# peterrum/deal-and-ceed-on-gpu

Measured on AMD Instinct MI355X. Metric: BP5 DoFs/sec per CG iter (p=4, ~1e8 DoFs) + % HBM roofline at 1/2/4/8 GPUs, higher is better.
Workload: dtype f64

## Files before the change

deal-and-ceed-on-gpu_amd/csrc/bp5_device.hpp:

```cpp
#pragma once
#include "bp5_internal.hpp"
#include "bp5_kernels.hpp"

#include <hip/hip_runtime.h>
#include <rccl/rccl.h>

#include <algorithm>
#include <cmath>
#include <cstdio>
#include <cstdlib>
#include <cstring>
#include <map>
#include <memory>
#include <tuple>
#include <vector>

using namespace bp5;

#define HIP_TRY(expr)                                                                                              \
  do {                                                                                                             \
    hipError_t e_ = (expr);                                                                                        \
    if (e_ != hipSuccess)                                                                                          \
      return fail(e_ == hipErrorNoDevice || e_ == hipErrorInvalidDevice ? BP5_ERR_NO_DEVICE : BP5_ERR_HIP,         \
                  std::string(#expr) + ": " + hipGetErrorString(e_));                                              \
// ... 776 lines not shown
      return fail(BP5_ERR_INVALID, "variant 59 needs the whole cell range"); }
    BP5_CASE(4, 57) { if (c0 == 0 && c1 == mf->n_cells) return LAUNCH_COLL(launch_block_t, 4, (32, BLK_SEQ), coef, src, dst, overwrite);
      return fail(BP5_ERR_INVALID, "variant 57 needs the whole cell range"); }
    BP5_CASE(4, 58) { if (c0 == 0 && c1 == mf->n_cells) return LAUNCH_COLL(launch_block_t, 4, (32, BLK_SINGLE | BLK_SEQ | BLK_NTM), coef, src, dst, overwrite);
      return fail(BP5_ERR_INVALID, "variant 58 needs the whole cell range"); }
#ifdef BP5_TIMING_BUILDS
    BP5_CASE(4, 99) return launch_block_t<4, false, 32, BLK_DEFAULT | BLK_STAMPS>(mf, call, coef, src, dst, true);
#endif
    BP5_CASE(4, 52) { if (c0 == 0 && c1 == mf->n_cells) return LAUNCH_COLL(launch_block_t, 4, (32, BLK_SINGLE), coef, src, dst, overwrite);
      return fail(BP5_ERR_INVALID, "variant 52 needs the whole cell range"); }
    BP5_CASE(4, 53) { if (c0 == 0 && c1 == mf->n_cells) return LAUNCH_COLL(launch_block_t, 4, (25, BLK_SINGLE), coef, src, dst, overwrite);
      return fail(BP5_ERR_INVALID, "variant 53 needs the whole cell range"); }
#ifdef BP5_TIMING_BUILDS
    BP5_CASE(4, 64) return launch_block_t<4, false, 32, BLK_DEFAULT | BLK_LATT>(mf, call, coef, src, dst, true);
    BP5_CASE(4, 65) return launch_block_t<4, false, 32, BLK_DEFAULT | BLK_LATT | 33554432>(mf, call, coef, src, dst, true);
    BP5_CASE(4, 66) return launch_block_t<4, false, 32, BLK_DEFAULT | BLK_LATT | 134217728>(mf, call, coef, src, dst, true);
    BP5_CASE(4, 87) return launch_block_t<4, false, 32, BLK_SINGLE | BLK_SEQ | BLK_RUNS | 65536>(mf, call, coef, src, dst, true);
    BP5_CASE(4, 91) return launch_block_t<4, false, 32, BLK_SINGLE | BLK_SEQ | BLK_RUNS | 1>(mf, call, coef, src, dst, true);
    BP5_CASE(4, 93) return launch_block_t<4, false, 32, BLK_SINGLE | BLK_SEQ | BLK_RUNS | 2>(mf, call, coef, src, dst, true);
    BP5_CASE(4, 95) return launch_block_t<4, false, 32, BLK_SINGLE | BLK_SEQ | BLK_RUNS | 4>(mf, call, coef, src, dst, true);
    BP5_CASE(4, 97) return launch_block_t<4, false, 32, BLK_STAMPS>(mf, call, coef, src, dst, true);
    BP5_CASE(4, 98) return launch_block_t<4, false, 32, BLK_STAMPS | BLK_SINGLE>(mf, call, coef, src, dst, true);
    BP5_CASE(4, 92) return launch_block_t<4, false, 32, BLK_SINGLE | 1>(mf, call, coef, src, dst, true);
    BP5_CASE(4, 96) return launch_block_t<4, false, 32, BLK_SINGLE | 5>(mf, call, coef, src, dst, true);
#endif
    BLOCK_CASE(5, 50, 36, 4, true);
    BLOCK_CASE(6, 50, 49, 4, false);
    BLOCK_CASE(7, 50, 64, 4, false);
    BLOCK_CASE(8, 50, 81, 4, false);
#ifdef BP5_TIMING_BUILDS
#define BABL_CASE(M) BP5_CASE(4, 60 + (M)) return launch_block_t<4, false, 25, M>(mf, call, coef, src, dst, true)
// ... 32 lines not shown
```

deal-and-ceed-on-gpu_amd/csrc/bp5_kernels.hpp:

```cpp
#pragma once
#include <hip/hip_runtime.h>
#include <stdint.h>
#include <type_traits>

namespace bp5 {

template <int n>
struct ShapeArg {
  double N[n * n];
  double D[n * n];
};

template <int n>
__host__ __device__ constexpr int coef_off(int qi, int ab)
{
  return (qi < 2 * (n / 2)) ? (qi / 2) * (2 * n * n) + 2 * ab + (qi & 1) : (n / 2) * (2 * n * n) + ab;
}
typedef double bp5_d2u __attribute__((ext_vector_type(2), aligned(8)));
template <int n, bool NT = false>
__device__ __forceinline__ void load_pencil(const double *base, int ab, double (&S)[n])
{
#pragma unroll
  for (int m = 0; m < n / 2; ++m) {
    const bp5_d2u *q = reinterpret_cast<const bp5_d2u *>(base + m * (2 * n * n) + 2 * ab);
    const bp5_d2u v = NT ? __builtin_nontemporal_load(q) : *q;
    S[2 * m] = v.x;
    S[2 * m + 1] = v.y;
  }
  if constexpr (n & 1) S[n - 1] = NT ? __builtin_nontemporal_load(base + (n / 2) * (2 * n * n) + ab) : base[(n / 2) * (2 * n * n) + ab];
}

typedef float bp5_f2u __attribute__((ext_vector_type(2), aligned(4)));
template <int n, bool NT = false>
__device__ __forceinline__ void load_pencil(const float *base, int ab, float (&S)[n])
{
#pragma unroll
  for (int m = 0; m < n / 2; ++m) {
    const bp5_f2u *q = reinterpret_cast<const bp5_f2u *>(base + m * (2 * n * n) + 2 * ab);
    const bp5_f2u v = NT ? __builtin_nontemporal_load(q) : *q;
    S[2 * m] = v.x;
    S[2 * m + 1] = v.y;
  }
  if constexpr (n & 1) S[n - 1] = NT ? __builtin_nontemporal_load(base + (n / 2) * (2 * n * n) + ab) : base[(n / 2) * (2 * n * n) + ab];
}
constexpr int BLK_F32M = 536870912;
template <int ABL> using metric_t = typename std::conditional<(ABL & BLK_F32M) != 0, float, double>::type;

template <int n, bool NT = false>
__device__ __forceinline__ void load_pencil_pair(const double *base, int ab, int m, double &s0, double &s1)
{
  const bp5_d2u *q = reinterpret_cast<const bp5_d2u *>(base + m * (2 * n * n) + 2 * ab);
  const bp5_d2u v = NT ? __builtin_nontemporal_load(q) : *q;
  s0 = v.x;
  s1 = v.y;
}
template <int n, bool NT = false>
__device__ __forceinline__ double load_pencil_tail(const double *base, int ab)
{
  return NT ? __builtin_nontemporal_load(base + (n / 2) * (2 * n * n) + ab) : base[(n / 2) * (2 * n * n) + ab];
}

struct ApplyArgs {
  const uint32_t *l2g;
  const double *coef;
  const double *src;
  double *dst;
  uint64_t plane_stride;
  uint64_t cell_stride;
  uint32_t cell_begin, cell_end;
  uint32_t n_teams;
  uint32_t teams_per_xcd;
  const double *gcell;
  uint32_t n_cells_total;
  const uint32_t *hang_mask;
// ... 203 lines not shown
#pragma unroll
  for (int k = 0; k < n; ++k) u[k] = (ABL & 4) ? 1e-9 * idx[k] : a.src[idx[k]];
  uint32_t hmask = 0;
  if constexpr ((ABL & 2097152) != 0) {
    hmask = a.hang_mask[cell];
    pencil_hang_resolve<n, TW, false, L>(hmask, a.hang_I, u, T, a_, b_, active);
  }

  if constexpr (ABL & 131072) {
    if (active) {
#pragma unroll
      for (int k = 0; k < n; ++k) a.dst[cell * n3 + k * n2 + abm] = u[k];
    }
  }
  using MT = metric_t<ABL>;
  const MT *cf = reinterpret_cast<const MT *>(a.coef) + cell * a.cell_stride;
  constexpr bool AFFINE = (ABL & 1024) != 0;
  constexpr bool HELM = (ABL & 8388608) != 0;
  static_assert(!HELM || (PF && !AFFINE), "Helmholtz build: prefetched planes, six-plane geometry");
  static_assert((ABL & BLK_F32M) == 0 || (!HELM && !AFFINE), "FP32 metric planes: Poisson operator, six-plane geometry");
  constexpr int NPL = HELM ? 7 : 6;
  MT S[(PF && !AFFINE) ? NPL : 1][n];
  double um[HELM ? n : 1];
  double Gc[6] = {0, 0, 0, 0, 0, 0};
  if constexpr (AFFINE) {
    load_pencil<n>(cf, abm, S[0]);
#pragma unroll
    for (int pl = 0; pl < 6; ++pl) Gc[pl] = a.gcell[(uint64_t)pl * a.n_cells_total + cell];
  } else if constexpr (PF) {
#pragma unroll
    for (int pl = 0; pl < NPL; ++pl) {
      if constexpr (ABL & 2) {
#pragma unroll
        for (int i = 0; i < n; ++i) S[pl][i] = 1.0 + pl + i + 1e-3 * abm;
      } else
        load_pencil<n, (ABL & 256) != 0>(cf + pl * a.plane_stride, abm, S[pl]);
    }
  }

  double g0[n], g1[n], g2[n];
  if constexpr (ABL & 8) {
#pragma unroll
    for (int i = 0; i < n; ++i) { g0[i] = u[i]; g1[i] = 2.0 * u[i]; g2[i] = 3.0 * u[i]; }
  } else if constexpr (!COLL) {
    double aN[n], aD[n];
    MV_N(sh.N, u, aN);
    MV_D(sh.D, u, aD);
    if (active) {
#pragma unroll
      for (int k = 0; k < n; ++k) { TL(0, k, b_, a_) = aN[k]; TL(1, k, b_, a_) = aD[k]; }
    }
    team_sync<TW>();
// ... 49 lines not shown
    if constexpr (HELM) {
#pragma unroll
      for (int i = 0; i < n; ++i) um[i] = r1[i];
    }
  }

#pragma unroll
  for (int i = 0; i < n; ++i) {
    double s00, s11, s22, s01, s02, s12;
    if constexpr (AFFINE) {
      const double sc = S[0][i];
      s00 = sc * Gc[0]; s11 = sc * Gc[1]; s22 = sc * Gc[2]; s01 = sc * Gc[3]; s02 = sc * Gc[4]; s12 = sc * Gc[5];
    } else if constexpr (PF) {
      s00 = S[0][i]; s11 = S[1][i]; s22 = S[2][i]; s01 = S[3][i]; s02 = S[4][i]; s12 = S[5][i];
    } else {
      s00 = cf[0 * a.plane_stride + coef_off<n>(i, abm)];
      s11 = cf[1 * a.plane_stride + coef_off<n>(i, abm)];
      s22 = cf[2 * a.plane_stride + coef_off<n>(i, abm)];
      s01 = cf[3 * a.plane_stride + coef_off<n>(i, abm)];
      s02 = cf[4 * a.plane_stride + coef_off<n>(i, abm)];
      s12 = cf[5 * a.plane_stride + coef_off<n>(i, abm)];
    }
    const double x0 = g0[i], x1 = g1[i], x2 = g2[i];
    g0[i] = s00 * x0 + s01 * x1 + s02 * x2;
    g1[i] = s01 * x0 + s11 * x1 + s12 * x2;
    g2[i] = s02 * x0 + s12 * x1 + s22 * x2;
    if constexpr (HELM) um[i] *= S[6][i];
  }

  double y[n];
  if constexpr (ABL & 8) {
#pragma unroll
    for (int i = 0; i < n; ++i) y[i] = g0[i] + g1[i] + g2[i];
  } else if constexpr (!COLL) {
    double e1[n], e2[n], e3[n];
    MV_DT(sh.D, g0, e1);
// ... 162 lines not shown

    uint32_t idx[n];
    double u[n];
    idx[0] = linked ? idx_carry : idxN[0];
    u[0] = linked ? u_carry : uN[0];
#pragma unroll
    for (int k = 1; k < n; ++k) { idx[k] = idxN[k]; u[k] = uN[k]; }
    u_carry = u[n - 1];
    idx_carry = idx[n - 1];
    {
      const uint32_t *l2g_n = a.l2g + (uint64_t)(e_next & 0x3fffffffu) * n3 + abm;
#pragma unroll
      for (int k = 0; k < n; ++k) idxN[k] = l2g_n[k * n2];
    }

    const double *cf = a.coef + cell * a.cell_stride;
    constexpr bool AFFINE = (ABL & 1024) != 0;
    double S[(PF && !AFFINE) ? 6 : 1][n];
    double Gc[6] = {0, 0, 0, 0, 0, 0};
    if constexpr (AFFINE) {
      load_pencil<n>(cf, abm, S[0]);
#pragma unroll
      for (int pl = 0; pl < 6; ++pl) Gc[pl] = a.gcell[(uint64_t)pl * a.n_cells_total + cell];
    } else if constexpr (PF) {
#pragma unroll
      for (int pl = 0; pl < 6; ++pl) {
        if constexpr (ABL & 2) {
#pragma unroll
          for (int i = 0; i < n; ++i) S[pl][i] = 1.0 + pl + i + 1e-3 * abm;
        } else
          load_pencil<n, (ABL & 256) != 0>(cf + pl * a.plane_stride, abm, S[pl]);
      }
    }

    double g0[n], g1[n], g2[n];
    if constexpr (ABL & 8) {
#pragma unroll
      for (int i = 0; i < n; ++i) { g0[i] = u[i]; g1[i] = 2.0 * u[i]; g2[i] = 3.0 * u[i]; }
    } else if constexpr (!COLL) {
      double aN[n], aD[n];
      MV_N(sh.N, u, aN);
      MV_D(sh.D, u, aD);
      if (active) {
#pragma unroll
        for (int k = 0; k < n; ++k) { TL(0, k, b_, a_) = aN[k]; TL(1, k, b_, a_) = aD[k]; }
      }
      team_sync<TW>();
// ... 47 lines not shown
      MV_D(sh.D, r1, g0);
    }

#pragma unroll
    for (int k = 0; k < n; ++k) uN[k] = a.src[idxN[k]];

#pragma unroll
    for (int i = 0; i < n; ++i) {
      double s00, s11, s22, s01, s02, s12;
      if constexpr (AFFINE) {
        const double sc = S[0][i];
        s00 = sc * Gc[0]; s11 = sc * Gc[1]; s22 = sc * Gc[2]; s01 = sc * Gc[3]; s02 = sc * Gc[4]; s12 = sc * Gc[5];
      } else if constexpr (PF) {
        s00 = S[0][i]; s11 = S[1][i]; s22 = S[2][i]; s01 = S[3][i]; s02 = S[4][i]; s12 = S[5][i];
      } else {
        s00 = cf[0 * a.plane_stride + coef_off<n>(i, abm)];
        s11 = cf[1 * a.plane_stride + coef_off<n>(i, abm)];
        s22 = cf[2 * a.plane_stride + coef_off<n>(i, abm)];
        s01 = cf[3 * a.plane_stride + coef_off<n>(i, abm)];
        s02 = cf[4 * a.plane_stride + coef_off<n>(i, abm)];
        s12 = cf[5 * a.plane_stride + coef_off<n>(i, abm)];
      }
      const double x0 = g0[i], x1 = g1[i], x2 = g2[i];
      g0[i] = s00 * x0 + s01 * x1 + s02 * x2;
      g1[i] = s01 * x0 + s11 * x1 + s12 * x2;
      g2[i] = s02 * x0 + s12 * x1 + s22 * x2;
    }

    double y[n];
    if constexpr (ABL & 8) {
#pragma unroll
      for (int i = 0; i < n; ++i) y[i] = g0[i] + g1[i] + g2[i];
    } else if constexpr (!COLL) {
      double e1[n], e2[n], e3[n];
      MV_DT(sh.D, g0, e1);
      MV_NT(sh.N, g1, e2);
// ... 106 lines not shown
  const int abm = ab < n2 ? ab : ab % n2;
  const int a_ = abm % n, b_ = abm / n;
  double *T = lds + (c < CPT ? c : 0) * L::CS;
#define TL(f, k, j, i) T[(f) * (n * L::PS) + (k) * L::PS + (j) * L::RS + (i)]

  const uint32_t o0 = tp.off[team];
  const int m = (int)(tp.off[team + 1] - o0);
  uint32_t gidx[MAXU];
#pragma unroll
  for (int r = 0; r < MAXU; ++r) {
    const int i = t + r * TEAM;
    gidx[r] = i < m ? tp.dofs[o0 + i] : 0u;
  }
  const int my_round = tp.cell_round[cell];
  const int n_rounds = tp.team_rounds[team];
  const double *cf = a.coef + cell * a.cell_stride;
  constexpr bool AFFINE = (ABL & 1024) != 0;
  double S[(PF && !AFFINE) ? 6 : 1][n];
  double Gc[6] = {0, 0, 0, 0, 0, 0};
  if constexpr (AFFINE) {
    load_pencil<n>(cf, abm, S[0]);
#pragma unroll
    for (int pl = 0; pl < 6; ++pl) Gc[pl] = a.gcell[(uint64_t)pl * a.n_cells_total + cell];
  } else if constexpr (PF) {
#pragma unroll
    for (int pl = 0; pl < 6; ++pl) load_pencil<n>(cf + pl * a.plane_stride, abm, S[pl]);
  }
  uint16_t ps[n];
  const uint16_t *pos_c = tp.pos + cell * n3 + abm;
#pragma unroll
  for (int k = 0; k < n; ++k) ps[k] = pos_c[k * n2];
  double u[n];
  if constexpr (ABL & 32) {
    const uint32_t *l2g_c = a.l2g + cell * n3 + abm;
    uint32_t idx[n];
#pragma unroll
    for (int k = 0; k < n; ++k) idx[k] = l2g_c[k * n2];
#pragma unroll
    for (int k = 0; k < n; ++k) u[k] = a.src[idx[k]];
  } else if constexpr (ABL & 4) {
#pragma unroll
// ... 59 lines not shown
    double r1[n];
#pragma unroll
    for (int i = 0; i < n; ++i) { r1[i] = TL(0, b_, a_, i); g1[i] = TL(1, b_, a_, i); g2[i] = TL(2, b_, a_, i); }
    MV_D(sh.D, r1, g0);
  }

#pragma unroll
  for (int i = 0; i < n; ++i) {
    double s00, s11, s22, s01, s02, s12;
    if constexpr (AFFINE) {
      const double sc = S[0][i];
      s00 = sc * Gc[0]; s11 = sc * Gc[1]; s22 = sc * Gc[2]; s01 = sc * Gc[3]; s02 = sc * Gc[4]; s12 = sc * Gc[5];
    } else if constexpr (PF) {
      s00 = S[0][i]; s11 = S[1][i]; s22 = S[2][i]; s01 = S[3][i]; s02 = S[4][i]; s12 = S[5][i];
    } else {
      s00 = cf[0 * a.plane_stride + coef_off<n>(i, abm)]; s11 = cf[1 * a.plane_stride + coef_off<n>(i, abm)]; s22 = cf[2 * a.plane_stride + coef_off<n>(i, abm)];
      s01 = cf[3 * a.plane_stride + coef_off<n>(i, abm)]; s02 = cf[4 * a.plane_stride + coef_off<n>(i, abm)]; s12 = cf[5 * a.plane_stride + coef_off<n>(i, abm)];
    }
    const double x0 = g0[i], x1 = g1[i], x2 = g2[i];
    g0[i] = s00 * x0 + s01 * x1 + s02 * x2;
    g1[i] = s01 * x0 + s11 * x1 + s12 * x2;
    g2[i] = s02 * x0 + s12 * x1 + s22 * x2;
  }

  double y[n];
  if constexpr (!COLL) {
    double e1[n], e2[n], e3[n];
    MV_DT(sh.D, g0, e1);
    MV_NT(sh.N, g1, e2);
    MV_NT(sh.N, g2, e3);
    __syncthreads();
    if (active) {
// ... 257 lines not shown
  {
    r.active = lane_ok && exists && !(r.ent >> 31);
    const uint64_t cell = r.ent & 0x7fffffffu;
    if constexpr (LATT) r.cpos = bp.cell_pos[cell];
    else if constexpr (PACK) load_pencil_idx<n, uint16_t>(bp.packed + cell * n3, abm, r.ps);
    else {
      load_pencil_idx<n, uint32_t>(bp.gidx + cell * n3, abm, r.idx);
      load_pencil_idx<n, uint16_t>(bp.pos + cell * n3, abm, r.ps);
    }
    r.round = bp.cell_round[cell];
    if constexpr (HANG) r.mask = a.hang_mask[cell];
    if constexpr (!SINGLE) issue_metric(a, r, abm);
  }
  static __device__ __forceinline__ void issue_metric_roll(const ApplyArgs &a, uint32_t ent, int abm, double (&S)[NPL][n])
  {
    const double *cf = a.coef + (uint64_t)(ent & 0x7fffffffu) * a.cell_stride;
#pragma unroll
    for (int pl = 0; pl < NPL; ++pl) {
      if constexpr (ABL & 2) {
#pragma unroll
        for (int i = 0; i < n; ++i) S[pl][i] = 1.0 + pl + i;
      } else
        load_pencil<n, (ABL & 32768) != 0>(cf + pl * a.plane_stride, abm, S[pl]);
    }
  }
  static __device__ __forceinline__ void issue_metric(const ApplyArgs &a, R &r, int abm)
  {
    if constexpr (ROLL) return;
    const uint64_t cell = r.ent & 0x7fffffffu;
    const MT *cf = reinterpret_cast<const MT *>(a.coef) + cell * a.cell_stride;
    if constexpr (AFFINE) {
      load_pencil<n>(cf, abm, r.S[0]);
#pragma unroll
      for (int pl = 0; pl < 6; ++pl) r.Gc[pl] = a.gcell[(uint64_t)pl * a.n_cells_total + cell];
    } else {
#ifdef BP5_TIMING_BUILDS
      if constexpr ((ABL & 33554432) != 0 && (n & 1)) {
        const uint64_t cell0 = (uint64_t)__builtin_amdgcn_readfirstlane((int)cell);
        const int lane = (int)(threadIdx.x & 63u);
#pragma unroll
        for (int pl = 0; pl < NPL; ++pl) {
          const double *base = a.coef + pl * a.plane_stride + ((cell0 * a.cell_stride) & ~(uint64_t)15);
#pragma unroll
          for (int m = 0; m < n / 2; ++m) {
            const bp5_d2u v = *reinterpret_cast<const bp5_d2u *>(base + (m * 64 + lane) * 2);
            r.S[pl][2 * m] = v.x;
            r.S[pl][2 * m + 1] = v.y;
          }
          r.S[pl][n - 1] = r.S[pl][0] + 1.0;
        }
        return;
      }
      if constexpr ((ABL & 134217728) != 0 && (n & 1) && NPL == 6) {
#pragma unroll
        for (int pl = 0; pl < NPL; ++pl) {
#pragma unroll
          for (int m = 0; m < n / 2; ++m) load_pencil_pair<n>(cf + pl * a.plane_stride, abm, m, r.S[pl][2 * m], r.S[pl][2 * m + 1]);
        }
#pragma unroll
        for (int pl = 0; pl < NPL; pl += 2) load_pencil_pair<n>(cf + pl * a.plane_stride, abm, n / 2, r.S[pl][n - 1], r.S[pl + 1][n - 1]);
        return;
      }
#endif
#pragma unroll
      for (int pl = 0; pl < NPL; ++pl) {
        if constexpr (ABL & 2) {
#pragma unroll
          for (int i = 0; i < n; ++i) r.S[pl][i] = 1.0 + pl + i;
        } else
          load_pencil<n, (ABL & 32768) != 0>(cf + pl * a.plane_stride, abm, r.S[pl]);
      }
    }
  }
  static __device__ __forceinline__ void decode_and_gather(const ApplyArgs &a, R &r, const uint32_t *rt, const double *staged = nullptr,
                                                           const uint32_t *lt = nullptr, int a_ = 0, int b_ = 0)
  {
    if constexpr (LATT) {
      const uint32_t hdr = lt[54];
      const int NXl = (int)(hdr & 255u) * P, NYl = (int)((hdr >> 8) & 255u) * P, NZl = (int)((hdr >> 16) & 255u) * P;
      const int I = (int)(r.cpos & 15u) * P + a_, J = (int)((r.cpos >> 4) & 15u) * P + b_, K0 = (int)(r.cpos >> 8) * P;
      const int eI = I == 0 ? 0 : I == NXl ? 2 : 1, eJ = J == 0 ? 0 : J == NYl ? 2 : 1;
      const uint32_t LX = eI == 1 ? (uint32_t)(NXl - 1) : 1u, LXY = LX * (eJ == 1 ? (uint32_t)(NYl - 1) : 1u);
      const uint32_t offIJ = (eI == 1 ? (uint32_t)(I - 1) : 0u) + LX * (eJ == 1 ? (uint32_t)(J - 1) : 0u);
      const int entIJ = eI + 3 * eJ;
#pragma unroll
      for (int k = 0; k < n; ++k) {
// ... 19 lines not shown
        const uint32_t dof = (rt[BLOCK_MAX_RUNS + run] & BLOCK_DOF_MASK) + off;
        r.u[k] = (ABL & 4) ? 1e-9 * dof : a.src[dof];
      }
    }
  }
  static __device__ __forceinline__ void issue_gather(const ApplyArgs &a, R &r)
  {
#pragma unroll
    for (int k = 0; k < n; ++k) r.u[k] = (ABL & 4) ? 1e-9 * r.idx[k] : a.src[r.idx[k]];
  }

  static __device__ __forceinline__ void run(const ApplyArgs &a, const ShapeArg<n> &sh, R &cur, R &nxt, double *T, double *acc, int a_, int b_,
                                             int n_rounds, int abm, unsigned long long (&ph)[8], unsigned long long &tprev, double &energy,
                                             double (&Sr)[ROLL ? NPL : 1][ROLL ? n : 1])
  {
    if constexpr (SINGLE && !ROLL) issue_metric(a, cur, abm);
    BP5_STAMP(0)
    if constexpr (SEQ) {
#define T1(k, j, i) T[(k) * L::PS + (j) * L::RS + (i)]
#define T2(k, j, i) T[(PP ? TILE_ONE : 0) + (k) * L::PS + (j) * L::RS + (i)]
      const bool act = cur.active;
      double(&uu)[n] = cur.u;
      bool hang_any = false;
      if constexpr (HANG) {
        const bool flagged = act && (cur.mask & BP5_HANG_ANY) != 0;
        if constexpr (WAVE_LOCAL) hang_any = __builtin_amdgcn_ballot_w64(flagged) != 0ull;
        else hang_any = __syncthreads_or(flagged) != 0;
        if (hang_any) pencil_hang_resolve<n, WAVE_LOCAL ? 1 : 4, false, L>(cur.mask, a.hang_I, uu, T, a_, b_, act);
      }
      double q0[n], q1[n], q2[n];
      double um[HELM ? n : 1];
      if constexpr (!COLL) {
        double aN[n], aD[n], vN[n], vD[n];
        MV_N(sh.N, uu, aN);
        MV_D(sh.D, uu, aD);
        if (act) {
#pragma unroll
          for (int k = 0; k < n; ++k) T1(k, b_, a_) = aN[k];
        }
        tile_sync();
#pragma unroll
        for (int j = 0; j < n; ++j) vN[j] = T1(b_, j, a_);
        tile_sync_r();
        if (act) {
// ... 83 lines not shown
          q1[i] = sc * (cur.Gc[3] * x0 + cur.Gc[1] * x1 + cur.Gc[5] * x2);
          q2[i] = sc * (cur.Gc[4] * x0 + cur.Gc[5] * x1 + cur.Gc[2] * x2);
        } else {
          q0[i] = SM(0) * x0 + SM(3) * x1 + SM(4) * x2;
          q1[i] = SM(3) * x0 + SM(1) * x1 + SM(5) * x2;
          q2[i] = SM(4) * x0 + SM(5) * x1 + SM(2) * x2;
        }
        if constexpr ((ABL & 1048576) != 0) { if (act) energy += x0 * q0[i] + x1 * q1[i] + x2 * q2[i]; }
        if constexpr (HELM) {
          const double uq = um[i];
          um[i] = SM(6) * uq;
          if constexpr ((ABL & 1048576) != 0) { if (act) energy += uq * um[i]; }
        }
      };
      if constexpr (ROLL) {
        const double *cfn = a.coef + (uint64_t)(nxt.ent & 0x7fffffffu) * a.cell_stride;
        constexpr bool NTM = (ABL & 32768) != 0;
#pragma unroll
        for (int m = 0; m < n / 2; ++m) {
          qpoint(2 * m, [&](int pl) { return Sr[pl][2 * m]; });
          qpoint(2 * m + 1, [&](int pl) { return Sr[pl][2 * m + 1]; });
          __builtin_amdgcn_sched_barrier(0);
          if constexpr (!(ABL & 2)) {
#pragma unroll
            for (int pl = 0; pl < NPL; ++pl) load_pencil_pair<n, NTM>(cfn + pl * a.plane_stride, abm, m, Sr[pl][2 * m], Sr[pl][2 * m + 1]);
          }
          __builtin_amdgcn_sched_barrier(0);
        }
        if constexpr (n & 1) {
          qpoint(n - 1, [&](int pl) { return Sr[pl][n - 1]; });
          __builtin_amdgcn_sched_barrier(0);
          if constexpr (!(ABL & 2)) {
#pragma unroll
            for (int pl = 0; pl < NPL; ++pl) Sr[pl][n - 1] = load_pencil_tail<n, NTM>(cfn + pl * a.plane_stride, abm);
          }
          __builtin_amdgcn_sched_barrier(0);
        }
      } else {
#pragma unroll
        for (int i = 0; i < n; ++i) qpoint(i, [&](int pl) { return cur.S[pl][i]; });
      }
      BP5_STAMP(3)
      double yy[n];
      if constexpr (!COLL) {
        double e1[n], e2[n], e3[n], w1[n], w2[n], w3[n];
        MV_DT(sh.D, q0, e1);
        if constexpr (HELM) MV_NT_ADD(sh.N, um, e1);
        MV_NT(sh.N, q1, e2);
        MV_NT(sh.N, q2, e3);
// ... 793 lines not shown
  const int q = i + n * (j + n * k);
  for (uint64_t cell = blockIdx.x; cell < n_cells; cell += gridDim.x) {
    const uint32_t g = l2g[cell * n3 + q];
    for (int e = 0; e < 3; ++e) X[e * n3 + q] = coords[3 * (uint64_t)g + e];
    __syncthreads();
    if (o.hang_mask)
      for (int e = 0; e < 3; ++e) hang_resolve3<n, false>(o.hang_mask[cell], o.hang_I, X + e * n3, t1, i, j, k);
    double J[3][3], K[3][3], xq[3];
    cell_jacobian<n>(tab, X, t1, t2, i, j, k, J, xq);
    const double det = invert3(J, K);
    const double *w = tab + 2 * n2;
    const double jxw = fabs(det) * w[i] * w[j] * w[k];
    if (o.coef) {
      const double kap = kappa_eval(kappa_mode, xq[0], xq[1], xq[2]);
      const double s = o.helmholtz ? jxw : jxw * kap;
      MT *c = reinterpret_cast<MT *>(o.coef) + cell * o.cell_stride + coef_off<n>(i, j + n * k);
      if (o.helmholtz) c[6 * o.plane_stride] = (MT)(jxw * kap);
      c[0 * o.plane_stride] = (MT)(s * (K[0][0] * K[0][0] + K[0][1] * K[0][1] + K[0][2] * K[0][2]));
      c[1 * o.plane_stride] = (MT)(s * (K[1][0] * K[1][0] + K[1][1] * K[1][1] + K[1][2] * K[1][2]));
      c[2 * o.plane_stride] = (MT)(s * (K[2][0] * K[2][0] + K[2][1] * K[2][1] + K[2][2] * K[2][2]));
      c[3 * o.plane_stride] = (MT)(s * (K[0][0] * K[1][0] + K[0][1] * K[1][1] + K[0][2] * K[1][2]));
      c[4 * o.plane_stride] = (MT)(s * (K[0][0] * K[2][0] + K[0][1] * K[2][1] + K[0][2] * K[2][2]));
      c[5 * o.plane_stride] = (MT)(s * (K[1][0] * K[2][0] + K[1][1] * K[2][1] + K[1][2] * K[2][2]));
    }
    if (o.scalar) {
      double Gq[6] = {K[0][0] * K[0][0] + K[0][1] * K[0][1] + K[0][2] * K[0][2], K[1][0] * K[1][0] + K[1][1] * K[1][1] + K[1][2] * K[1][2],
                      K[2][0] * K[2][0] + K[2][1] * K[2][1] + K[2][2] * K[2][2], K[0][0] * K[1][0] + K[0][1] * K[1][1] + K[0][2] * K[1][2],
                      K[0][0] * K[2][0] + K[0][1] * K[2][1] + K[0][2] * K[2][2], K[1][0] * K[2][0] + K[1][1] * K[2][1] + K[1][2] * K[2][2]};
      o.scalar[cell * n3 + coef_off<n>(i, j + n * k)] = jxw * kappa_eval(kappa_mode, xq[0], xq[1], xq[2]);
      for (int c6 = 0; c6 < 6; ++c6) {
        if (q == 0) { t1[c6] = Gq[c6]; o.gcell[(uint64_t)c6 * o.n_cells + cell] = Gq[c6]; }
      }
      __syncthreads();
      double dev = 0.0, nrm = 0.0;
      for (int c6 = 0; c6 < 6; ++c6) { dev = fmax(dev, fabs(Gq[c6] - t1[c6])); nrm = fmax(nrm, fabs(t1[c6])); }
      t2[q] = dev / nrm;
      __syncthreads();
      if (q == 0) {
// ... 11 lines not shown
      for (int e = 0; e < 3; ++e) o.q_points[(uint64_t)e * o.geo_plane + at] = xq[e];
    }
    __syncthreads();
  }
}

template <int n, typename MT = double>
__global__ void metric_permute_kernel(const MT *in, double *out, uint64_t total , uint64_t n_cells, uint64_t plane_stride,
                                      uint64_t cell_stride)
{
  constexpr int n2 = n * n, n3 = n2 * n;
  for (uint64_t o = blockIdx.x * (uint64_t)blockDim.x + threadIdx.x; o < total; o += (uint64_t)gridDim.x * blockDim.x) {
    const uint64_t cellplane = o / n3, plane = cellplane / n_cells, cell = cellplane - plane * n_cells;
    const int q = (int)(o - cellplane * n3);
    const int qi = q % n, rest = q / n;
    out[o] = in[plane * plane_stride + cell * cell_stride + coef_off<n>(qi, rest)];
  }
}

template <int n>
__global__ void __launch_bounds__(n *n *n) rhs_kernel(const uint32_t *l2g, const double *coords, const double *tab_gauss,
                                                     uint32_t n_cells, double *b, const uint32_t *hang_mask, const double *hang_I)
{
  constexpr int n2 = n * n, n3 = n2 * n;
  __shared__ double X[3 * n3], t1[n3], t2[n3], v[n3];
  const int i = threadIdx.x, j = threadIdx.y, k = threadIdx.z;
  const int q = i + n * (j + n * k);
  for (uint64_t cell = blockIdx.x; cell < n_cells; cell += gridDim.x) {
    const uint32_t g = l2g[cell * n3 + q];
    for (int e = 0; e < 3; ++e) X[e * n3 + q] = coords[3 * (uint64_t)g + e];
    __syncthreads();
// ... 24 lines not shown
{
  constexpr int n2 = n * n, n3 = n2 * n;
  __shared__ double S[n3], t1[n3], t2[n3], NN[n2], DD[n2], ND[n2];
  const int i = threadIdx.x, j = threadIdx.y, k = threadIdx.z;
  const int q = i + n * (j + n * k);
  if (q < n2) {
    const double a = tab[q], b = tab[n2 + q];
    NN[q] = a * a;
    DD[q] = b * b;
    ND[q] = a * b;
  }
  __syncthreads();
  for (uint64_t cell = blockIdx.x; cell < n_cells; cell += gridDim.x) {
    double acc = 0.0;
    for (int c = 0; c < n_planes; ++c) {
      const uint64_t at = cell * (gcell ? (uint64_t)n3 : cell_stride) + coef_off<n>(i, j + n * k);
      S[q] = gcell ? coef[at] * gcell[(uint64_t)c * n_cells + cell] : coef[(uint64_t)c * plane_stride + at];
      __syncthreads();
      const double *X = (c == 0) ? DD : (c == 3 || c == 4) ? ND : NN;
      const double *Y = (c == 1) ? DD : (c == 3 || c == 5) ? ND : NN;
      const double *Z = (c == 2) ? DD : (c == 4 || c == 5) ? ND : NN;
      const double y = Cell3<n>::template tensor3<true>(X, Y, Z, S, t1, t2, i, j, k);
      acc += (c < 3 || c == 6) ? y : 2.0 * y;
    }
    const uint32_t hm = hang_mask ? hang_mask[cell] : 0u;
    const bool coarse_entry = (hm & BP5_HANG_ANY) && (hang_on_line(hm, 0, i, j, k, n - 1) || hang_on_line(hm, 1, i, j, k, n - 1) || hang_on_line(hm, 2, i, j, k, n - 1));
    if (!coarse_entry) atomic_add_f64(diag + l2g[cell * n3 + q], acc);
  }
}

template <int n>
__global__ void __launch_bounds__(n *n *n) diagonal_hanging_kernel(const uint32_t *l2g, const double *coef, uint64_t plane_stride, uint64_t cell_stride, const double *gcell,
                                                                  const double *tab, uint32_t n_cells, double *diag, const uint32_t *hang_mask,
                                                                  const double *hang_I)
{
  constexpr int n2 = n * n, n3 = n2 * n;
  __shared__ double v[n3], w[n3], t1[n3], t2[n3];
  const int i = threadIdx.x, j = threadIdx.y, k = threadIdx.z;
  const int q = i + n * (j + n * k);
  const double *N = tab, *D = tab + n2;
  for (uint64_t cell = blockIdx.x; cell < n_cells; cell += gridDim.x) {
    const uint32_t hm = hang_mask[cell];
    if (!(hm & BP5_HANG_ANY)) continue;
    double S[6];
    const uint64_t at = cell * cell_stride + coef_off<n>(i, j + n * k);
#pragma unroll
    for (int c = 0; c < 6; ++c) S[c] = gcell ? coef[at] * gcell[(uint64_t)c * n_cells + cell] : coef[(uint64_t)c * plane_stride + at];
    for (int s = 0; s < n3; ++s) {
      const int si = s % n, sj = (s / n) % n, sk = s / n2;
      if (!(hang_on_line(hm, 0, si, sj, sk, n - 1) || hang_on_line(hm, 1, si, sj, sk, n - 1) || hang_on_line(hm, 2, si, sj, sk, n - 1))) continue;
      v[q] = q == s ? 1.0 : 0.0;
      __syncthreads();
      hang_resolve3<n, false>(hm, hang_I, v, t1, i, j, k);
      const double g0 = Cell3<n>::template tensor3<false>(D, N, N, v, t1, t2, i, j, k);
      const double g1 = Cell3<n>::template tensor3<false>(N, D, N, v, t1, t2, i, j, k);
      const double g2 = Cell3<n>::template tensor3<false>(N, N, D, v, t1, t2, i, j, k);
      const double h0 = S[0] * g0 + S[3] * g1 + S[4] * g2, h1 = S[3] * g0 + S[1] * g1 + S[5] * g2, h2 = S[4] * g0 + S[5] * g1 + S[2] * g2;
      w[q] = h0;
      __syncthreads();
      double y = Cell3<n>::template tensor3<true>(D, N, N, w, t1, t2, i, j, k);
      w[q] = h1;
      __syncthreads();
// ... 1137 lines not shown
```

Before: 27.80 billion.

## Interleave odd-degree metric plane pairs so pencil tails load as pairs

After: 27.90 billion (median of 6 runs). About the same (+0.4%).

```diff
diff --git a/deal-and-ceed-on-gpu_amd/csrc/bp5_device.hpp b/deal-and-ceed-on-gpu_amd/csrc/bp5_device.hpp
--- a/deal-and-ceed-on-gpu_amd/csrc/bp5_device.hpp
+++ b/deal-and-ceed-on-gpu_amd/csrc/bp5_device.hpp
@@ -814,7 +814,6 @@
 #ifdef BP5_TIMING_BUILDS
     BP5_CASE(4, 64) return launch_block_t<4, false, 32, BLK_DEFAULT | BLK_LATT>(mf, call, coef, src, dst, true);
     BP5_CASE(4, 65) return launch_block_t<4, false, 32, BLK_DEFAULT | BLK_LATT | 33554432>(mf, call, coef, src, dst, true);
-    BP5_CASE(4, 66) return launch_block_t<4, false, 32, BLK_DEFAULT | BLK_LATT | 134217728>(mf, call, coef, src, dst, true);
     BP5_CASE(4, 87) return launch_block_t<4, false, 32, BLK_SINGLE | BLK_SEQ | BLK_RUNS | 65536>(mf, call, coef, src, dst, true);
     BP5_CASE(4, 91) return launch_block_t<4, false, 32, BLK_SINGLE | BLK_SEQ | BLK_RUNS | 1>(mf, call, coef, src, dst, true);
     BP5_CASE(4, 93) return launch_block_t<4, false, 32, BLK_SINGLE | BLK_SEQ | BLK_RUNS | 2>(mf, call, coef, src, dst, true);
diff --git a/deal-and-ceed-on-gpu_amd/csrc/bp5_kernels.hpp b/deal-and-ceed-on-gpu_amd/csrc/bp5_kernels.hpp
--- a/deal-and-ceed-on-gpu_amd/csrc/bp5_kernels.hpp
+++ b/deal-and-ceed-on-gpu_amd/csrc/bp5_kernels.hpp
@@ -16,48 +16,99 @@
 {
   return (qi < 2 * (n / 2)) ? (qi / 2) * (2 * n * n) + 2 * ab + (qi & 1) : (n / 2) * (2 * n * n) + ab;
 }
+template <int n>
+__host__ __device__ constexpr bool coef_paired(int pl)
+{
+  return (n & 1) && pl < 6;
+}
+template <int n>
+__host__ __device__ constexpr uint64_t coef_plane_base(int pl, uint64_t plane_stride)
+{
+  return (uint64_t)(coef_paired<n>(pl) ? pl & ~1 : pl) * plane_stride;
+}
+template <int n>
+__host__ __device__ constexpr uint64_t coef_cell_step(int pl, uint64_t cell_stride)
+{
+  return coef_paired<n>(pl) && cell_stride == (uint64_t)(n * n * n) ? (uint64_t)(2 * n * n * n) : cell_stride;
+}
+template <int n>
+__host__ __device__ constexpr uint64_t coef_chunk(int pl, uint64_t cell, uint64_t plane_stride, uint64_t cell_stride)
+{
+  return coef_plane_base<n>(pl, plane_stride) + cell * coef_cell_step<n>(pl, cell_stride);
+}
+template <int n>
+__host__ __device__ constexpr int coef_in(int pl, int qi, int ab)
+{
+  return !coef_paired<n>(pl) ? coef_off<n>(qi, ab) : qi < n - 1 ? (pl & 1) * (n - 1) * n * n + coef_off<n>(qi, ab) : 2 * (n - 1) * n * n + 2 * ab + (pl & 1);
+}
+static_assert(coef_in<5>(2, 4, 7) + 1 == coef_in<5>(3, 4, 7) && coef_in<5>(3, 2, 7) + 1 == coef_in<5>(3, 3, 7) && coef_in<4>(3, 2, 7) == coef_off<4>(2, 7), "pairs are neighbours");
+
 typedef double bp5_d2u __attribute__((ext_vector_type(2), aligned(8)));
-template <int n, bool NT = false>
-__device__ __forceinline__ void load_pencil(const double *base, int ab, double (&S)[n])
-{
-#pragma unroll
-  for (int m = 0; m < n / 2; ++m) {
-    const bp5_d2u *q = reinterpret_cast<const bp5_d2u *>(base + m * (2 * n * n) + 2 * ab);
-    const bp5_d2u v = NT ? __builtin_nontemporal_load(q) : *q;
-    S[2 * m] = v.x;
-    S[2 * m + 1] = v.y;
-  }
-  if constexpr (n & 1) S[n - 1] = NT ? __builtin_nontemporal_load(base + (n / 2) * (2 * n * n) + ab) : base[(n / 2) * (2 * n * n) + ab];
-}
-
 typedef float bp5_f2u __attribute__((ext_vector_type(2), aligned(4)));
-template <int n, bool NT = false>
-__device__ __forceinline__ void load_pencil(const float *base, int ab, float (&S)[n])
-{
-#pragma unroll
-  for (int m = 0; m < n / 2; ++m) {
-    const bp5_f2u *q = reinterpret_cast<const bp5_f2u *>(base + m * (2 * n * n) + 2 * ab);
-    const bp5_f2u v = NT ? __builtin_nontemporal_load(q) : *q;
-    S[2 * m] = v.x;
-    S[2 * m + 1] = v.y;
-  }
-  if constexpr (n & 1) S[n - 1] = NT ? __builtin_nontemporal_load(base + (n / 2) * (2 * n * n) + ab) : base[(n / 2) * (2 * n * n) + ab];
-}
+template <bool NT, typename MT>
+__device__ __forceinline__ void load_two(const MT *p, MT &s0, MT &s1)
+{
+  using V = typename std::conditional<std::is_same<MT, float>::value, bp5_f2u, bp5_d2u>::type;
+  const V *q = reinterpret_cast<const V *>(p);
+  const V v = NT ? __builtin_nontemporal_load(q) : *q;
+  s0 = v.x;
+  s1 = v.y;
+}
+template <int n, bool NT = false, typename MT>
+__device__ __forceinline__ void load_pencil(const MT *base, int ab, MT (&S)[n])
+{
+#pragma unroll
+  for (int m = 0; m < n / 2; ++m) load_two<NT>(base + coef_off<n>(2 * m, ab), S[2 * m], S[2 * m + 1]);
+  if constexpr (n & 1) S[n - 1] = NT ? __builtin_nontemporal_load(base + coef_off<n>(n - 1, ab)) : base[coef_off<n>(n - 1, ab)];
+}
+
 constexpr int BLK_F32M = 536870912;
 template <int ABL> using metric_t = typename std::conditional<(ABL & BLK_F32M) != 0, float, double>::type;
 
-template <int n, bool NT = false>
-__device__ __forceinline__ void load_pencil_pair(const double *base, int ab, int m, double &s0, double &s1)
-{
-  const bp5_d2u *q = reinterpret_cast<const bp5_d2u *>(base + m * (2 * n * n) + 2 * ab);
-  const bp5_d2u v = NT ? __builtin_nontemporal_load(q) : *q;
-  s0 = v.x;
-  s1 = v.y;
-}
-template <int n, bool NT = false>
-__device__ __forceinline__ double load_pencil_tail(const double *base, int ab)
-{
-  return NT ? __builtin_nontemporal_load(base + (n / 2) * (2 * n * n) + ab) : base[(n / 2) * (2 * n * n) + ab];
+template <int n, typename MT>
+struct MetricCell {
+  const MT *coef, *cell0;
+  uint64_t cell, plane_stride, cell_stride;
+  __device__ __forceinline__ const MT *chunk(int pl) const
+  {
+    return pl < 6 ? cell0 + coef_plane_base<n>(pl, plane_stride) : coef + coef_chunk<n>(pl, cell, plane_stride, cell_stride);
+  }
+  __device__ __forceinline__ MT at(int pl, int qi, int ab) const { return chunk(pl)[coef_in<n>(pl, qi, ab)]; }
+  template <bool NT = false>
+  __device__ __forceinline__ void pair(int pl, int ab, int m, MT &s0, MT &s1) const
+  {
+    load_two<NT>(chunk(pl) + coef_in<n>(pl, 2 * m, ab), s0, s1);
+  }
+  template <bool NT = false>
+  __device__ __forceinline__ MT tail(int pl, int ab) const
+  {
+    const MT *p = chunk(pl) + coef_in<n>(pl, n - 1, ab);
+    return NT ? __builtin_nontemporal_load(p) : *p;
+  }
+  template <bool NT = false>
+  __device__ __forceinline__ void tails(int c, int ab, MT &t0, MT &t1) const
+  {
+    load_two<NT>(chunk(c) + coef_in<n>(c, n - 1, ab), t0, t1);
+  }
+  template <int NPL, bool NT = false>
+  __device__ __forceinline__ void load(int ab, MT (&S)[NPL][n]) const
+  {
+#pragma unroll
+    for (int pl = 0; pl < NPL; ++pl) {
+#pragma unroll
+      for (int m = 0; m < n / 2; ++m) pair<NT>(pl, ab, m, S[pl][2 * m], S[pl][2 * m + 1]);
+      if constexpr (n & 1) {
+        if (!coef_paired<n>(pl)) S[pl][n - 1] = tail<NT>(pl, ab);
+        else if (pl & 1) tails<NT>(pl - 1, ab, S[pl - 1][n - 1], S[pl][n - 1]);
+      }
+    }
+  }
+};
+template <int n, typename MT>
+__device__ __forceinline__ MetricCell<n, MT> metric_cell(const MT *coef, uint64_t cell, uint64_t plane_stride, uint64_t cell_stride)
+{
+  asm volatile("" : "+s"(plane_stride));
+  return MetricCell<n, MT>{coef, coef + coef_chunk<n>(0, cell, plane_stride, cell_stride), cell, plane_stride, cell_stride};
 }
 
 struct ApplyArgs {
@@ -291,7 +342,7 @@
     }
   }
   using MT = metric_t<ABL>;
-  const MT *cf = reinterpret_cast<const MT *>(a.coef) + cell * a.cell_stride;
+  const auto mc = metric_cell<n>(reinterpret_cast<const MT *>(a.coef), cell, a.plane_stride, a.cell_stride);
   constexpr bool AFFINE = (ABL & 1024) != 0;
   constexpr bool HELM = (ABL & 8388608) != 0;
   static_assert(!HELM || (PF && !AFFINE), "Helmholtz build: prefetched planes, six-plane geometry");
@@ -301,18 +352,18 @@
   double um[HELM ? n : 1];
   double Gc[6] = {0, 0, 0, 0, 0, 0};
   if constexpr (AFFINE) {
-    load_pencil<n>(cf, abm, S[0]);
+    load_pencil<n>(mc.coef + cell * a.cell_stride, abm, S[0]);
 #pragma unroll
     for (int pl = 0; pl < 6; ++pl) Gc[pl] = a.gcell[(uint64_t)pl * a.n_cells_total + cell];
   } else if constexpr (PF) {
-#pragma unroll
-    for (int pl = 0; pl < NPL; ++pl) {
-      if constexpr (ABL & 2) {
+    if constexpr (ABL & 2) {
+#pragma unroll
+      for (int pl = 0; pl < NPL; ++pl) {
 #pragma unroll
         for (int i = 0; i < n; ++i) S[pl][i] = 1.0 + pl + i + 1e-3 * abm;
-      } else
-        load_pencil<n, (ABL & 256) != 0>(cf + pl * a.plane_stride, abm, S[pl]);
-    }
+      }
+    } else
+      mc.template load<NPL, (ABL & 256) != 0>(abm, S);
   }
 
   double g0[n], g1[n], g2[n];
@@ -392,12 +443,12 @@
     } else if constexpr (PF) {
       s00 = S[0][i]; s11 = S[1][i]; s22 = S[2][i]; s01 = S[3][i]; s02 = S[4][i]; s12 = S[5][i];
     } else {
-      s00 = cf[0 * a.plane_stride + coef_off<n>(i, abm)];
-      s11 = cf[1 * a.plane_stride + coef_off<n>(i, abm)];
-      s22 = cf[2 * a.plane_stride + coef_off<n>(i, abm)];
-      s01 = cf[3 * a.plane_stride + coef_off<n>(i, abm)];
-      s02 = cf[4 * a.plane_stride + coef_off<n>(i, abm)];
-      s12 = cf[5 * a.plane_stride + coef_off<n>(i, abm)];
+      s00 = mc.at(0, i, abm);
+      s11 = mc.at(1, i, abm);
+      s22 = mc.at(2, i, abm);
+      s01 = mc.at(3, i, abm);
+      s02 = mc.at(4, i, abm);
+      s12 = mc.at(5, i, abm);
     }
     const double x0 = g0[i], x1 = g1[i], x2 = g2[i];
     g0[i] = s00 * x0 + s01 * x1 + s02 * x2;
@@ -590,23 +641,23 @@
       for (int k = 0; k < n; ++k) idxN[k] = l2g_n[k * n2];
     }
 
-    const double *cf = a.coef + cell * a.cell_stride;
+    const auto mc = metric_cell<n>(a.coef, cell, a.plane_stride, a.cell_stride);
     constexpr bool AFFINE = (ABL & 1024) != 0;
     double S[(PF && !AFFINE) ? 6 : 1][n];
     double Gc[6] = {0, 0, 0, 0, 0, 0};
     if constexpr (AFFINE) {
-      load_pencil<n>(cf, abm, S[0]);
+      load_pencil<n>(mc.coef + cell * a.cell_stride, abm, S[0]);
 #pragma unroll
       for (int pl = 0; pl < 6; ++pl) Gc[pl] = a.gcell[(uint64_t)pl * a.n_cells_total + cell];
     } else if constexpr (PF) {
-#pragma unroll
-      for (int pl = 0; pl < 6; ++pl) {
-        if constexpr (ABL & 2) {
+      if constexpr (ABL & 2) {
+#pragma unroll
+        for (int pl = 0; pl < 6; ++pl) {
 #pragma unroll
           for (int i = 0; i < n; ++i) S[pl][i] = 1.0 + pl + i + 1e-3 * abm;
-        } else
-          load_pencil<n, (ABL & 256) != 0>(cf + pl * a.plane_stride, abm, S[pl]);
-      }
+        }
+      } else
+        mc.template load<6, (ABL & 256) != 0>(abm, S);
     }
 
     double g0[n], g1[n], g2[n];
@@ -684,12 +735,12 @@
       } else if constexpr (PF) {
         s00 = S[0][i]; s11 = S[1][i]; s22 = S[2][i]; s01 = S[3][i]; s02 = S[4][i]; s12 = S[5][i];
       } else {
-        s00 = cf[0 * a.plane_stride + coef_off<n>(i, abm)];
-        s11 = cf[1 * a.plane_stride + coef_off<n>(i, abm)];
-        s22 = cf[2 * a.plane_stride + coef_off<n>(i, abm)];
-        s01 = cf[3 * a.plane_stride + coef_off<n>(i, abm)];
-        s02 = cf[4 * a.plane_stride + coef_off<n>(i, abm)];
-        s12 = cf[5 * a.plane_stride + coef_off<n>(i, abm)];
+        s00 = mc.at(0, i, abm);
+        s11 = mc.at(1, i, abm);
+        s22 = mc.at(2, i, abm);
+        s01 = mc.at(3, i, abm);
+        s02 = mc.at(4, i, abm);
+        s12 = mc.at(5, i, abm);
       }
       const double x0 = g0[i], x1 = g1[i], x2 = g2[i];
       g0[i] = s00 * x0 + s01 * x1 + s02 * x2;
@@ -826,17 +877,16 @@
   }
   const int my_round = tp.cell_round[cell];
   const int n_rounds = tp.team_rounds[team];
-  const double *cf = a.coef + cell * a.cell_stride;
+  const auto mc = metric_cell<n>(a.coef, cell, a.plane_stride, a.cell_stride);
   constexpr bool AFFINE = (ABL & 1024) != 0;
   double S[(PF && !AFFINE) ? 6 : 1][n];
   double Gc[6] = {0, 0, 0, 0, 0, 0};
   if constexpr (AFFINE) {
-    load_pencil<n>(cf, abm, S[0]);
+    load_pencil<n>(mc.coef + cell * a.cell_stride, abm, S[0]);
 #pragma unroll
     for (int pl = 0; pl < 6; ++pl) Gc[pl] = a.gcell[(uint64_t)pl * a.n_cells_total + cell];
   } else if constexpr (PF) {
-#pragma unroll
-    for (int pl = 0; pl < 6; ++pl) load_pencil<n>(cf + pl * a.plane_stride, abm, S[pl]);
+    mc.template load<6>(abm, S);
   }
   uint16_t ps[n];
   const uint16_t *pos_c = tp.pos + cell * n3 + abm;
@@ -926,8 +976,8 @@
     } else if constexpr (PF) {
       s00 = S[0][i]; s11 = S[1][i]; s22 = S[2][i]; s01 = S[3][i]; s02 = S[4][i]; s12 = S[5][i];
     } else {
-      s00 = cf[0 * a.plane_stride + coef_off<n>(i, abm)]; s11 = cf[1 * a.plane_stride + coef_off<n>(i, abm)]; s22 = cf[2 * a.plane_stride + coef_off<n>(i, abm)];
-      s01 = cf[3 * a.plane_stride + coef_off<n>(i, abm)]; s02 = cf[4 * a.plane_stride + coef_off<n>(i, abm)]; s12 = cf[5 * a.plane_stride + coef_off<n>(i, abm)];
+      s00 = mc.at(0, i, abm); s11 = mc.at(1, i, abm); s22 = mc.at(2, i, abm);
+      s01 = mc.at(3, i, abm); s02 = mc.at(4, i, abm); s12 = mc.at(5, i, abm);
     }
     const double x0 = g0[i], x1 = g1[i], x2 = g2[i];
     g0[i] = s00 * x0 + s01 * x1 + s02 * x2;
@@ -1215,23 +1265,22 @@
   }
   static __device__ __forceinline__ void issue_metric_roll(const ApplyArgs &a, uint32_t ent, int abm, double (&S)[NPL][n])
   {
-    const double *cf = a.coef + (uint64_t)(ent & 0x7fffffffu) * a.cell_stride;
-#pragma unroll
-    for (int pl = 0; pl < NPL; ++pl) {
-      if constexpr (ABL & 2) {
+    if constexpr (ABL & 2) {
+#pragma unroll
+      for (int pl = 0; pl < NPL; ++pl) {
 #pragma unroll
         for (int i = 0; i < n; ++i) S[pl][i] = 1.0 + pl + i;
-      } else
-        load_pencil<n, (ABL & 32768) != 0>(cf + pl * a.plane_stride, abm, S[pl]);
-    }
+      }
+    } else
+      metric_cell<n>(a.coef, (uint64_t)(ent & 0x7fffffffu), a.plane_stride, a.cell_stride).template load<NPL, (ABL & 32768) != 0>(abm, S);
   }
   static __device__ __forceinline__ void issue_metric(const ApplyArgs &a, R &r, int abm)
   {
     if constexpr (ROLL) return;
     const uint64_t cell = r.ent & 0x7fffffffu;
-    const MT *cf = reinterpret_cast<const MT *>(a.coef) + cell * a.cell_stride;
+    const auto mc = metric_cell<n>(reinterpret_cast<const MT *>(a.coef), cell, a.plane_stride, a.cell_stride);
     if constexpr (AFFINE) {
-      load_pencil<n>(cf, abm, r.S[0]);
+      load_pencil<n>(mc.coef + cell * a.cell_stride, abm, r.S[0]);
 #pragma unroll
       for (int pl = 0; pl < 6; ++pl) r.Gc[pl] = a.gcell[(uint64_t)pl * a.n_cells_total + cell];
     } else {
@@ -1252,25 +1301,15 @@
         }
         return;
       }
-      if constexpr ((ABL & 134217728) != 0 && (n & 1) && NPL == 6) {
+#endif
+      if constexpr (ABL & 2) {
 #pragma unroll
         for (int pl = 0; pl < NPL; ++pl) {
 #pragma unroll
-          for (int m = 0; m < n / 2; ++m) load_pencil_pair<n>(cf + pl * a.plane_stride, abm, m, r.S[pl][2 * m], r.S[pl][2 * m + 1]);
-        }
-#pragma unroll
-        for (int pl = 0; pl < NPL; pl += 2) load_pencil_pair<n>(cf + pl * a.plane_stride, abm, n / 2, r.S[pl][n - 1], r.S[pl + 1][n - 1]);
-        return;
-      }
-#endif
-#pragma unroll
-      for (int pl = 0; pl < NPL; ++pl) {
-        if constexpr (ABL & 2) {
-#pragma unroll
           for (int i = 0; i < n; ++i) r.S[pl][i] = 1.0 + pl + i;
-        } else
-          load_pencil<n, (ABL & 32768) != 0>(cf + pl * a.plane_stride, abm, r.S[pl]);
-      }
+        }
+      } else
+        mc.template load<NPL, (ABL & 32768) != 0>(abm, r.S);
     }
   }
   static __device__ __forceinline__ void decode_and_gather(const ApplyArgs &a, R &r, const uint32_t *rt, const double *staged = nullptr,
@@ -1320,7 +1359,8 @@
                                              int n_rounds, int abm, unsigned long long (&ph)[8], unsigned long long &tprev, double &energy,
                                              double (&Sr)[ROLL ? NPL : 1][ROLL ? n : 1])
   {
-    if constexpr (SINGLE && !ROLL) issue_metric(a, cur, abm);
+    constexpr bool METRIC_LATE = HANG && COLL;
+    if constexpr (SINGLE && !ROLL && !METRIC_LATE) issue_metric(a, cur, abm);
     BP5_STAMP(0)
     if constexpr (SEQ) {
 #define T1(k, j, i) T[(k) * L::PS + (j) * L::RS + (i)]
@@ -1334,6 +1374,7 @@
         else hang_any = __syncthreads_or(flagged) != 0;
         if (hang_any) pencil_hang_resolve<n, WAVE_LOCAL ? 1 : 4, false, L>(cur.mask, a.hang_I, uu, T, a_, b_, act);
       }
+      if constexpr (SINGLE && !ROLL && METRIC_LATE) issue_metric(a, cur, abm);
       double q0[n], q1[n], q2[n];
       double um[HELM ? n : 1];
       if constexpr (!COLL) {
@@ -1447,7 +1488,7 @@
         }
       };
       if constexpr (ROLL) {
-        const double *cfn = a.coef + (uint64_t)(nxt.ent & 0x7fffffffu) * a.cell_stride;
+        const auto mcn = metric_cell<n>(a.coef, (uint64_t)(nxt.ent & 0x7fffffffu), a.plane_stride, a.cell_stride);
         constexpr bool NTM = (ABL & 32768) != 0;
 #pragma unroll
         for (int m = 0; m < n / 2; ++m) {
@@ -1456,7 +1497,7 @@
           __builtin_amdgcn_sched_barrier(0);
           if constexpr (!(ABL & 2)) {
 #pragma unroll
-            for (int pl = 0; pl < NPL; ++pl) load_pencil_pair<n, NTM>(cfn + pl * a.plane_stride, abm, m, Sr[pl][2 * m], Sr[pl][2 * m + 1]);
+            for (int pl = 0; pl < NPL; ++pl) mcn.template pair<NTM>(pl, abm, m, Sr[pl][2 * m], Sr[pl][2 * m + 1]);
           }
           __builtin_amdgcn_sched_barrier(0);
         }
@@ -1465,7 +1506,10 @@
           __builtin_amdgcn_sched_barrier(0);
           if constexpr (!(ABL & 2)) {
 #pragma unroll
-            for (int pl = 0; pl < NPL; ++pl) Sr[pl][n - 1] = load_pencil_tail<n, NTM>(cfn + pl * a.plane_stride, abm);
+            for (int pl = 0; pl < NPL; ++pl) {
+              if (!coef_paired<n>(pl)) Sr[pl][n - 1] = mcn.template tail<NTM>(pl, abm);
+              else if (pl & 1) mcn.template tails<NTM>(pl - 1, abm, Sr[pl - 1][n - 1], Sr[pl][n - 1]);
+            }
           }
           __builtin_amdgcn_sched_barrier(0);
         }
@@ -2289,14 +2333,15 @@
     if (o.coef) {
       const double kap = kappa_eval(kappa_mode, xq[0], xq[1], xq[2]);
       const double s = o.helmholtz ? jxw : jxw * kap;
-      MT *c = reinterpret_cast<MT *>(o.coef) + cell * o.cell_stride + coef_off<n>(i, j + n * k);
-      if (o.helmholtz) c[6 * o.plane_stride] = (MT)(jxw * kap);
-      c[0 * o.plane_stride] = (MT)(s * (K[0][0] * K[0][0] + K[0][1] * K[0][1] + K[0][2] * K[0][2]));
-      c[1 * o.plane_stride] = (MT)(s * (K[1][0] * K[1][0] + K[1][1] * K[1][1] + K[1][2] * K[1][2]));
-      c[2 * o.plane_stride] = (MT)(s * (K[2][0] * K[2][0] + K[2][1] * K[2][1] + K[2][2] * K[2][2]));
-      c[3 * o.plane_stride] = (MT)(s * (K[0][0] * K[1][0] + K[0][1] * K[1][1] + K[0][2] * K[1][2]));
-      c[4 * o.plane_stride] = (MT)(s * (K[0][0] * K[2][0] + K[0][1] * K[2][1] + K[0][2] * K[2][2]));
-      c[5 * o.plane_stride] = (MT)(s * (K[1][0] * K[2][0] + K[1][1] * K[2][1] + K[1][2] * K[2][2]));
+      MT *const cf = reinterpret_cast<MT *>(o.coef);
+      auto c = [&](int pl) -> MT & { return cf[coef_chunk<n>(pl, cell, o.plane_stride, o.cell_stride) + coef_in<n>(pl, i, j + n * k)]; };
+      if (o.helmholtz) c(6) = (MT)(jxw * kap);
+      c(0) = (MT)(s * (K[0][0] * K[0][0] + K[0][1] * K[0][1] + K[0][2] * K[0][2]));
+      c(1) = (MT)(s * (K[1][0] * K[1][0] + K[1][1] * K[1][1] + K[1][2] * K[1][2]));
+      c(2) = (MT)(s * (K[2][0] * K[2][0] + K[2][1] * K[2][1] + K[2][2] * K[2][2]));
+      c(3) = (MT)(s * (K[0][0] * K[1][0] + K[0][1] * K[1][1] + K[0][2] * K[1][2]));
+      c(4) = (MT)(s * (K[0][0] * K[2][0] + K[0][1] * K[2][1] + K[0][2] * K[2][2]));
+      c(5) = (MT)(s * (K[1][0] * K[2][0] + K[1][1] * K[2][1] + K[1][2] * K[2][2]));
     }
     if (o.scalar) {
       double Gq[6] = {K[0][0] * K[0][0] + K[0][1] * K[0][1] + K[0][2] * K[0][2], K[1][0] * K[1][0] + K[1][1] * K[1][1] + K[1][2] * K[1][2],
@@ -2338,7 +2383,7 @@
     const uint64_t cellplane = o / n3, plane = cellplane / n_cells, cell = cellplane - plane * n_cells;
     const int q = (int)(o - cellplane * n3);
     const int qi = q % n, rest = q / n;
-    out[o] = in[plane * plane_stride + cell * cell_stride + coef_off<n>(qi, rest)];
+    out[o] = in[coef_chunk<n>((int)plane, cell, plane_stride, cell_stride) + coef_in<n>((int)plane, qi, rest)];
   }
 }
 
@@ -2393,8 +2438,8 @@
   for (uint64_t cell = blockIdx.x; cell < n_cells; cell += gridDim.x) {
     double acc = 0.0;
     for (int c = 0; c < n_planes; ++c) {
-      const uint64_t at = cell * (gcell ? (uint64_t)n3 : cell_stride) + coef_off<n>(i, j + n * k);
-      S[q] = gcell ? coef[at] * gcell[(uint64_t)c * n_cells + cell] : coef[(uint64_t)c * plane_stride + at];
+      S[q] = gcell ? coef[cell * n3 + coef_off<n>(i, j + n * k)] * gcell[(uint64_t)c * n_cells + cell]
+                   : coef[coef_chunk<n>(c, cell, plane_stride, cell_stride) + coef_in<n>(c, i, j + n * k)];
       __syncthreads();
       const double *X = (c == 0) ? DD : (c == 3 || c == 4) ? ND : NN;
       const double *Y = (c == 1) ? DD : (c == 3 || c == 5) ? ND : NN;
@@ -2422,9 +2467,10 @@
     const uint32_t hm = hang_mask[cell];
     if (!(hm & BP5_HANG_ANY)) continue;
     double S[6];
-    const uint64_t at = cell * cell_stride + coef_off<n>(i, j + n * k);
-#pragma unroll
-    for (int c = 0; c < 6; ++c) S[c] = gcell ? coef[at] * gcell[(uint64_t)c * n_cells + cell] : coef[(uint64_t)c * plane_stride + at];
+#pragma unroll
+    for (int c = 0; c < 6; ++c)
+      S[c] = gcell ? coef[cell * n3 + coef_off<n>(i, j + n * k)] * gcell[(uint64_t)c * n_cells + cell]
+                   : coef[coef_chunk<n>(c, cell, plane_stride, cell_stride) + coef_in<n>(c, i, j + n * k)];
     for (int s = 0; s < n3; ++s) {
       const int si = s % n, sj = (s / n) % n, sk = s / n2;
       if (!(hang_on_line(hm, 0, si, sj, sk, n - 1) || hang_on_line(hm, 1, si, sj, sk, n - 1) || hang_on_line(hm, 2, si, sj, sk, n - 1))) continue;
```
